# phecda-xu/FullyCNNSpeechEnhancement

Measured on AMD Instinct MI355X. Metric: spectrogram frames/sec (CR-CED-16 fwd, 129-bin), higher is better.
Workload: dtype f32; 1 GPU; CR-CED V3 (16-layer, skip connections) forward, batch 256 per GPU, 129x512, fp32 (BASELINE configs[2]); variant=FullyCNNV3, batch_per_gpu=256, frames=512, bins=129, global_batch=256, fused_available=True, parallelism=batch-shard x1, rccl_world_size=1, weights=random-init (glorot, seed 42), library=rced-hip 0.1 gfx950

## Files before the change

fullycnnspeechenhancement_amd/csrc/kernels_fused_v3.h:

```cpp
#pragma once
#include <hip/hip_runtime.h>

#include <type_traits>

#include "lds_dma.h"

#ifndef RCED_V3_LEGACY_FORMS
#define RCED_V3_LEGACY_FORMS 0
#endif
#ifndef RCED_D1
#define RCED_D1 1
#endif
#ifndef RCED_D2
#define RCED_D2 2
#endif
#ifndef RCED_D2X
#define RCED_D2X 1
#endif
#ifndef RCED_D3
#define RCED_D3 2
#endif
#ifndef RCED_LANE_OPAQUE
#define RCED_LANE_OPAQUE 1
#endif
// ... 1168 lines not shown
  constexpr int kPadPairs = 64 * kHS / 2;
#pragma unroll
  for (int i = 0; i < (5 * kPadPairs + kThreads - 1) / kThreads; ++i) {
    const int q = tid + i * kThreads, p = q / kPadPairs, e = q - p * kPadPairs;
    if (q < 5 * kPadPairs) lds_st<f32x2>(lds0 + 4 * (M::kHOff + p * kHFrame * kHS + 2 * e), 0, f32x2{0.f, 0.f});
  }
}
typedef f32x4 __attribute__((aligned(4))) f32x4_u;
template <int CTRL>
__device__ __forceinline__ float row_dpp(float v) {
  return __builtin_bit_cast(float, __builtin_amdgcn_update_dpp(0, __builtin_bit_cast(int, v), CTRL, 0xf, 0xf, true));
}

template <class M>
__device__ __forceinline__ void final_phase(const Params& P, unsigned lds0, unsigned w128, int wave, int lane, int utt,
                                            int t0, const FinA& A, const XStage& xnext, float* x0) {
  lane = opaque(lane);
  const int n = lane & 15, kq = lane >> 4;
  const f32x4 zero4 = {0.f, 0.f, 0.f, 0.f};
  float* yt = P.y + ((size_t)utt * P.T + t0) * kF;
  const int nfr = P.T - t0 < kTF ? P.T - t0 : kTF;
  if (wave == 2) {
    const int fi = kq, sub = n;
    const unsigned hb = lds0 + 4 * (M::kHOff + (kHFrame * fi + 64 + 64 + sub) * kHS);
    const unsigned wb = w128 + sub * 32;
    f32x4 hv[5][2], wv[5][2];
#pragma unroll
    for (int m = 0; m < 5; ++m)
#pragma unroll
      for (int c = 0; c < 2; ++c) {
        const f32x2 h0 = lds_ld<f32x2>(hb, (16 * m * kHS + 4 * c) * 4), h1 = lds_ld<f32x2>(hb, (16 * m * kHS + 4 * c + 2) * 4);
        hv[m][c] = f32x4{h0.x, h0.y, h1.x, h1.y};
        wv[m][c] = lds_ld<f32x4>(wb, (16 * m * 8 + 4 * c) * 4);
      }
    f32x4 s4 = {0.f, 0.f, 0.f, 0.f};
#pragma unroll
    for (int m = 0; m < 5; ++m)
#pragma unroll
      for (int c = 0; c < 2; ++c) {
        s4.x = __builtin_fmaf(hv[m][c].x, wv[m][c].x, s4.x);
        s4.y = __builtin_fmaf(hv[m][c].y, wv[m][c].y, s4.y);
        s4.z = __builtin_fmaf(hv[m][c].z, wv[m][c].z, s4.z);
        s4.w = __builtin_fmaf(hv[m][c].w, wv[m][c].w, s4.w);
      }
    float sum = (s4.x + s4.y) + (s4.z + s4.w);
    sum += row_dpp<0xB1>(sum);
    sum += row_dpp<0x4E>(sum);
    sum += row_dpp<0x141>(sum);
    sum += row_dpp<0x140>(sum);
    if (sub == 0 && fi < nfr) yt[fi * kF + 128] = sum + P.fin_bias;
  }
  {
    const unsigned rd0 = lds0 + 4 * (M::kHOff + ((kHFrame * (n >> 2) + 16 * (n & 3)) * kHS + 2 * kq)) + wave * (kFinRun * kHS * 4);
    unsigned rd1 = rd0 + 64 * kHS * 4;
    asm volatile("" : "+v"(rd1));
    f32x4 acc[2][2] = {{zero4, zero4}, {zero4, zero4}};
    constexpr int D = 2, RING = D + 1;
    f32x2 b[RING][2];
    run_job<kFinRun, D>(
        [&](auto ic) {
          constexpr int i = decltype(ic)::value, r = i % RING;
          b[r][0] = lds_ld<f32x2>(rd0, i * kHS * 4);
          b[r][1] = lds_ld<f32x2>(rd1, i * kHS * 4);
        },
        [&](auto ic) {
          constexpr int i = decltype(ic)::value, r = i % RING;
          acc[0][0] = mfma(A.a[i].x, b[r][0].x, acc[0][0]);
          acc[1][0] = mfma(A.a[i].x, b[r][1].x, acc[1][0]);
          acc[0][1] = mfma(A.a[i].y, b[r][0].y, acc[0][1]);
          acc[1][1] = mfma(A.a[i].y, b[r][1].y, acc[1][1]);
        },
        [] {});
    const unsigned scr = lds0 + M::finscr0(wave) + lane * 16;
    lds_st<f32x4>(scr, 0, acc[0][0] + acc[0][1]);
    lds_st<f32x4>(scr, M::kFinScrCt, acc[1][0] + acc[1][1]);
  }
  xstage_store(xnext, x0, wave * 64 + lane);
  __syncthreads();
  if (wave < 2) {
    const unsigned scr = lds0 + wave * M::kFinScrCt + lane * 16;
    f32x4 v = lds_ld<f32x4>(scr, M::finscr0(0));
#pragma unroll
    for (int w = 1; w < kWaves; ++w) v += lds_ld<f32x4>(scr, M::finscr0(w));
    v += f32x4{P.fin_bias, P.fin_bias, P.fin_bias, P.fin_bias};
    const int fi = n >> 2, f0 = 16 * (4 * wave + (n & 3)) + 4 * kq;
    if (fi < nfr) {
      *reinterpret_cast<f32x4_u*>(yt + fi * kF + f0) = v;
      store_wait_state();
    }
  } else if (wave == 3 && !M::kFused) {
    if constexpr (M::kX6) {
      constexpr int kRows = kB18Pad + 4 * kTF;
#pragma unroll
      for (int i = 0; i < (3 * kRows * 2 + 63) / 64; ++i) {
        const int q = lane + 64 * i, pl = q / (kRows * 2), e = q - pl * (kRows * 2), rr = e >> 1, half = e & 1;
        const int row = rr < kB18Pad ? rr : kB18Pad + kF + kS * ((rr - kB18Pad) >> 2) + ((rr - kB18Pad) & 3);
        if (q < 3 * kRows * 2) lds_st<f32x4>(lds0 + 4 * M::kB18Off + pl * M::kPlaneBytes + row * 32 + half * 16, 0, zero4);
      }
    } else {
      constexpr int kGapPairs = 4 * 18 / 2;
#pragma unroll
      for (int i = 0; i < (4 * kGapPairs + 63) / 64; ++i) {
        const int q = lane + 64 * i, g = q / kGapPairs, e = q - g * kGapPairs;
        if (q < 4 * kGapPairs)
          lds_st<f32x2>(lds0 + 4 * (M::kB18Off + (kB18Pad + kF + kS * g) * 18 + 2 * e), 0, f32x2{0.f, 0.f});
      }
    }
  }
}

#include "kernels_fused_v3_allx6.h"

template <class M>
__global__ __launch_bounds__(RCED_V3_LB) __attribute__((target("no-packed-fp32-ops"))) void fused_v3_kernel(Params P) {
  extern __shared__ __attribute__((aligned(16))) float lds[];
  const int tid = threadIdx.x;
  const int lane = tid & 63;
  const int wave = __builtin_amdgcn_readfirstlane(tid >> 6);
  float* const wbase = lds + M::kWOff;
#define WREG(i) (wbase + (i) * kWRegion)

  for (int e = tid; e < M::kLdsFloats; e += kThreads) lds[e] = 0.f;
  __syncthreads();
  A1Regs A1;
  A2Regs A2;
  const wrsrc_t wrs = __builtin_amdgcn_make_buffer_rsrc(const_cast<float*>(P.wpack), 0, (M::kAllX6 ? kATotal : M::kFused ? kTTotal : M::kX6 ? kGTotal : kWTotal) * 4, 0x00020000);
  constexpr bool kL1X = M::kFused && RCED_T_L1X6;
  auto wload = [&](auto kc, int g, unsigned voff, int g1size = kG1) {
    constexpr int k = decltype(kc)::value;
    if constexpr (k < 7) a1_load_one<k>(A1, wrs, g, voff);
    else if constexpr (k < 17) a2_load_one<k - 7>(A2, wrs, g + g1size, RCED_L2_BOTH ? 0 : wave >> 2, voff);
  };
  if constexpr (M::kAllX6) {
    packet_dma<kFinTFloats>(P.fin, lds + M::kFinTOff, wave, lane);
    a1x_dma<M>(P.wpack, lds, wave, lane);
  } else if constexpr (M::kX6) {
    const unsigned voff = (unsigned)lane * 16u;
    static_for<0, 7>([&](auto kc) { wload(kc, 0, voff); });
    if constexpr (M::kFused) packet_dma<kFin128>(P.fin + kFinA, lds + M::kFin128Off, wave, lane);
  } else {
    packet_dma<kW1>(P.wpack, WREG(0), wave, lane);
  }
  int wcur = 0;
  unsigned epoch = 0;
  const int tiles_base = P.total_tiles / (int)gridDim.x, tiles_rem = P.total_tiles % (int)gridDim.x;
  const int tile_begin = (int)blockIdx.x * tiles_base + ((int)blockIdx.x < tiles_rem ? (int)blockIdx.x : tiles_rem);
  const int tile_end = tile_begin + tiles_base + ((int)blockIdx.x < tiles_rem ? 1 : 0);
  XStage xst = xstage_load(P, tile_begin < tile_end ? tile_begin : P.total_tiles, tid);
#if RCED_STAMPS
  unsigned long long tsum[8] = {0, 0, 0, 0, 0, 0, 0, 0}, tfin = 0, tdet[16] = {0, 0, 0, 0, 0, 0, 0, 0, 0, 0, 0, 0, 0, 0, 0, 0};
#endif
  layer_end_sync();

  const int w1 = M::kFused && RCED_T_L1SWAP ? wave ^ 4 : wave;
  const int xr0 = w1 == 7 ? 3 : w1 - 4;
#ifdef RCED_PRIO
  if ((wave >= 4) == (RCED_PRIO > 0)) __builtin_amdgcn_s_setprio(1);
#endif
  const Lane L = make_lane<M>(lds, wave, lane, xr0 < 0 ? 0 : xr0, w1);
  const unsigned lds0 = lds_addr(lds);
  xstage_store(xst, lds + M::kX0Off, tid);
  __syncthreads();
  if constexpr (M::kAllX6) {
    convert_x0<M>(lds0, wave, lane);
    __syncthreads();
  }
  constexpr int kBlockFloats = M::kFused ? kTBlock : M::kX6 ? kGBlock : kWBlock;

  for (int tile = tile_begin; tile < tile_end; ++tile) {
    const int utt = tile / P.tiles_per_utt;
    const int t0 = (tile - utt * P.tiles_per_utt) * kTF;
    f32x4 skip_ce1[3], skip_ce2[3];
#pragma unroll
    for (int t = 0; t < 3; ++t) skip_ce1[t] = skip_ce2[t] = f32x4{0.f, 0.f, 0.f, 0.f};
    f32x2 sk1[5], sk2[5];
#pragma unroll
    for (int t = 0; t < 5; ++t) sk1[t] = sk2[t] = f32x2{0.f, 0.f};
    const float* wsrc = P.wpack;
    int gofs = 0;

    auto l1_section = [&](auto whichc, int blk) __attribute__((always_inline)) {
      constexpr int which = decltype(whichc)::value;
      {
        STAMP_BEGIN();
        const unsigned wb = lds_addr(WREG(wcur));
        auto dma = [&] {
          if constexpr (M::kFused) packet_dma<kG2 + kW3T>(wsrc + (M::kAllX6 ? kG1A : kL1X && blk > 0 ? kG1X : kG1), WREG(0), wave, lane);
          else if constexpr (M::kX6) packet_dma<kW3>(wsrc + kG1 + kG2, WREG(0), wave, lane);
          else packet_dma<kW2>(wsrc + kW1, WREG(wcur ^ 1), wave, lane);
        };
        A1Rem A1r;
        const unsigned voff1 = (unsigned)opaque(lane) * 16u;
        auto sp1 = [&](auto kc) {
          constexpr int k = decltype(kc)::value;
          if constexpr (M::kX6 && !(RCED_X6_EXP & 2)) {
            if constexpr (k >= 10) a1_load_rem_one<k - 10>(A1r, wrs, gofs, voff1);
            else if constexpr (!M::kFused || ((RCED_T_A2REG == 1 || RCED_T_A2REG == 2) && k < 9)) wload(IC<k + 7>{}, gofs, voff1);
          }
        };
        auto late = [&] {
          if constexpr (M::kX6 && (!M::kFused || RCED_T_A2REG == 2) && RCED_L2_BOTH && !(RCED_X6_EXP & 2))
            static_for<0, 10>([&](auto kc) { a2_load_one<decltype(kc)::value, kL2MT - 1>(A2, wrs, gofs + kG1, 1, voff1); });
        };
        auto sp1x = [&](auto kc) {
          constexpr int k = decltype(kc)::value;
          if constexpr (kL1X && k >= 12 && k < 21 && (RCED_T_A2REG == 1 || RCED_T_A2REG == 2)) wload(IC<k - 12 + 7>{}, gofs, voff1, M::kAllX6 ? kG1A : kG1X);
        };
        if constexpr (kL1X) {
          if constexpr (which == 1) layer1<M, true>(L, wb, A1, A1r, w1, dma, sp1, late DET_PASS);
          else layer1_x6l<M>(L, lds0, w1, dma, sp1x DET_PASS);
        } else {
          if (blk == 0) layer1<M, true>(L, wb, A1, A1r, w1, dma, sp1, late DET_PASS);
          else layer1<M, false>(L, wb, A1, A1r, w1, dma, sp1, late DET_PASS);
        }

        if constexpr (!M::kX6) wcur ^= 1;
#if RCED_STAMPS
        const unsigned long long st_b_ = stamp();
        tsum[blk == 0 ? 6 : 0] += st_b_ - st_a_;
        layer_end_sync();
        tsum[blk == 0 ? 7 : 3] += stamp() - st_b_;
#else
        layer_end_sync();
#endif
        if constexpr (!M::kFused) {
          STAMP_BEGIN();
          const unsigned tag2 = 0xC0000000u | (epoch + 1u);
          if constexpr (M::kX6) {
#if RCED_V3_LEGACY_FORMS
            if constexpr (RCED_L2_BOTH) layer2_x6_both<M>(L, lds0, A2, wave, tag2, P.err, [] {} DET_PASS);
            else layer2_x6<M>(L, lds0, A2, wave, tag2, P.err, [] {} DET_PASS);
#else
            static_assert(!M::kX6 || M::kFused, "form 1 is a legacy form (RCED_V3_LEGACY_FORMS)");
#endif
          } else {
            auto dma3 = [&] { packet_dma<kW3>(wsrc + kW1 + kW2, WREG(wcur ^ 1), wave, lane); };
            layer2_f32<M>(L, lds0, lds_addr(WREG(wcur)), wave, tag2, P.err, dma3 DET_PASS);
            wcur ^= 1;
          }
          STAMP_MATH(1);
          layer_end_sync();
          STAMP_WAIT(1);
        }
            }
    };
    if constexpr (M::kAllX6) l1_section(IC<0>{}, 0);
    else if constexpr (kL1X) l1_section(IC<1>{}, 0);
#pragma unroll 1
    for (int blk = 0;; ++blk) {
      if constexpr (kL1X) {
        if (blk > 0) l1_section(IC<0>{}, blk);
      } else {
        l1_section(IC<2>{}, blk);
      }
      if (blk == 4) break;
      if constexpr (M::kFused) {
        STAMP_BEGIN();
        ++epoch;
        const unsigned voff = (unsigned)opaque(lane) * 16u;
        auto sp = [&](auto jc) {
          constexpr int j = decltype(jc)::value;
          if constexpr (!kL1X) {
            if constexpr (2 * j < 7) wload(IC<2 * j>{}, gofs + kBlockFloats, voff);
            if constexpr (2 * j + 1 < 7) wload(IC<2 * j + 1>{}, gofs + kBlockFloats, voff);
          }
        };
        auto dma1 = [&] {
          if constexpr (kL1X) a1x_dma<M>(wsrc + (M::kAllX6 ? kTBlockA : blk == 0 ? kTBlock : kTBlockX), lds, wave, lane);
        };
        layer23<M, false>(P, L, lds0, lds_addr(WREG(0)), A2, blk, wave, 0x80000000u | epoch, sk1, sk2, sp, dma1 DET_PASS);
        STAMP_MATH(2);
        layer_end_sync();
        STAMP_WAIT(2);
      } else {
        STAMP_BEGIN();
        const unsigned wb = lds_addr(WREG(M::kX6 ? 0 : wcur));
        ++epoch;
        const unsigned tag = 0x80000000u | epoch;
        const float* wnext = wsrc + kBlockFloats;
        auto dma = [&] {
          if constexpr (!M::kX6) packet_dma<kW1>(wnext, WREG(wcur ^ 1), wave, lane);
        };
        const unsigned voff = (unsigned)opaque(lane) * 16u;
        auto sp = [&](auto kc) {
          if constexpr (M::kX6 && !(RCED_X6_EXP & 4) && decltype(kc)::value < 7) wload(kc, gofs + kBlockFloats, voff);
        };
        layer3<M, false>(P, L, lds0, wb, blk, wave, tag, skip_ce1, skip_ce2, dma, sp DET_PASS);
        if constexpr (!M::kX6) wcur ^= 1;
        STAMP_MATH(2);
        layer_end_sync();
        STAMP_WAIT(2);
      }
      wsrc += M::kAllX6 ? kTBlockA : kL1X && blk > 0 ? kTBlockX : kBlockFloats;
      gofs += M::kAllX6 ? kTBlockA : kL1X && blk > 0 ? kTBlockX : kBlockFloats;
    }
    FinA finA;
    if constexpr (M::kAllX6) {
      STAMP_BEGIN();
      ++epoch;
      xst = xstage_load(P, tile + 1 < tile_end ? tile + 1 : P.total_tiles, tid);
      if (wave == 0 && lane < 3) lds_st<u32x4>(lds0 + 4 * M::kB8Off + kHZeroRow * 16 + (unsigned)lane * kHPlaneBytes, 0, u32x4{0u, 0u, 0u, 0u});
      auto dma1 = [&] { a1x_dma<M>(P.wpack, lds, wave, lane); };
      layer23<M, true>(P, L, lds0, lds_addr(WREG(0)), A2, 4, wave, 0x80000000u | epoch, sk1, sk2, [](auto) {}, dma1 DET_PASS);
      STAMP_MATH(2);
      layer_end_sync();
      STAMP_WAIT(2);
    } else if constexpr (M::kFused) {
      STAMP_BEGIN();
      ++epoch;
      xst = xstage_load(P, tile + 1 < tile_end ? tile + 1 : P.total_tiles, tid);
      const int lane_o = opaque(lane);
      auto sp = [&](auto jc) {
        constexpr int j = decltype(jc)::value, s0 = (kFinRun * j) / 5, s1 = (kFinRun * (j + 1)) / 5;
        const f32x2* src = reinterpret_cast<const f32x2*>(P.fin) + (size_t)(kFinRun * wave) * 64 + lane_o;
#pragma unroll
        for (int q = s0; q < s1; ++q) finA.a[q] = src[q * 64];
      };
      layer23<M, true>(P, L, lds0, lds_addr(WREG(0)), A2, 4, wave, 0x80000000u | epoch, sk1, sk2, sp, [] {} DET_PASS);
      STAMP_MATH(2);
      layer_end_sync();
      STAMP_WAIT(2);
      const unsigned voff = (unsigned)opaque(lane) * 16u;
      static_for<0, 7>([&](auto kc) { wload(kc, 0, voff); });
    } else {
      STAMP_BEGIN();
      const unsigned wb = lds_addr(WREG(M::kX6 ? 0 : wcur));
      ++epoch;
      const unsigned tag = 0x80000000u | epoch;
      xst = xstage_load(P, tile + 1 < tile_end ? tile + 1 : P.total_tiles, tid);
      if constexpr (M::kX6) packet_dma<kFin128>(P.fin + kFinA, lds + M::kFin128Off, wave, lane);
      else packet_dma<kFin128>(P.fin + kFinA, WREG(wcur ^ 1) + kW1, wave, lane);
      fin_prefetch(P, wave, lane, finA);
      fin_zero_pads<M>(lds0, tid);
      auto dma = [&] {
        if constexpr (!M::kX6) packet_dma<kW1>(P.wpack, WREG(wcur ^ 1), wave, lane);
      };
      const unsigned voff = (unsigned)opaque(lane) * 16u;
      auto sp = [&](auto kc) {
        if constexpr (M::kX6 && !(RCED_X6_EXP & 4) && decltype(kc)::value < 7) wload(kc, 0, voff);
      };
      layer3<M, true>(P, L, lds0, wb, 4, wave, tag, skip_ce1, skip_ce2, dma, sp DET_PASS);
      if constexpr (!M::kX6) wcur ^= 1;
      STAMP_MATH(2);
      layer_end_sync();
      STAMP_WAIT(2);
    }
#if RCED_STAMPS
    const unsigned long long st_f_ = stamp();
#endif
    if constexpr (M::kAllX6) {
      final_phase_x6<M>(P, lds0, wave, lane, utt, t0, xst, lds + M::kX0Off DET_PASS);
    } else {
      const unsigned w128 = M::kX6 ? lds0 + 4 * M::kFin128Off : lds_addr(WREG(wcur) + kW1);
      final_phase<M>(P, lds0, w128, wave, lane, utt, t0, finA, xst, lds + M::kX0Off);
    }
#if RCED_STAMPS
    tfin += stamp() - st_f_;
#endif
  }
#undef WREG
#if RCED_STAMPS
  if (P.stamps && blockIdx.x == 0 && lane == 0)
    for (int i = 0; i < 8; ++i) P.stamps[wave * 8 + i] = tsum[i];
  if (P.stamps && blockIdx.x == 0 && lane == 0) P.stamps[64 + wave * 3] = tfin;
  if (P.stamps && blockIdx.x == 0 && lane == 0)
    for (int i = 0; i < 16; ++i) P.stamps[88 + wave * 16 + i] = tdet[i];
#endif
}


}
}
```

fullycnnspeechenhancement_amd/csrc/kernels_fused_v3_allx6.h:

```cpp
#pragma once

template <class M>
__device__ __forceinline__ void convert_px(unsigned lds0, int i, int f) {
  const unsigned src = lds0 + 4 * (M::kX0Off + 4 + i * kS + f);
  float v[8];
#pragma unroll
  for (int rr = 0; rr < 8; ++rr) v[rr] = lds_ld<float>(src, rr * kS * 4);
  u32x4 h, m, l;
#pragma unroll
  for (int q = 0; q < 4; ++q) {
    const P3 p = split2(v[2 * q], v[2 * q + 1]);
    h[q] = p.h;
    m[q] = p.m;
    l[q] = p.l;
  }
  const unsigned dst = lds0 + 4 * M::kB8Off + (kB8Pad + i * kS + f) * 16;
  lds_st<u32x4>(dst, 0, h);
  lds_st<u32x4>(dst, kB8PlaneBytes, m);
  lds_st<u32x4>(dst, 2 * kB8PlaneBytes, l);
}
template <class M>
__device__ __forceinline__ void convert_x0(unsigned lds0, int wave, int lane) {
  lane = opaque(lane);
  const int tid = wave * 64 + lane;
  convert_px<M>(lds0, tid >> 7, tid & 127);
  if (wave == 7 && lane < kTF) convert_px<M>(lds0, lane, kF - 1);
  const int z = tid - 5 * 64;
  if (z >= 0 && z < 72) {
    const int part = z / 24, rr = z - part * 24;
    const int row = rr < 4 ? rr : rr < 20 ? kB8Pad + kS * ((rr - 4) >> 2) + kF + ((rr - 4) & 3) : kB8Pad + kNPX + (rr - 20);
    lds_st<u32x4>(lds0 + 4 * M::kB8Off + part * kB8PlaneBytes + row * 16, 0, u32x4{0u, 0u, 0u, 0u});
  }
}
static_assert(kB8Rows == kB8Pad + kNPX + 4, "convert_x0 zeroes the planes' pad, gap and trailing rows by this map");

template <class M, int NCH, bool CT2ALL>
__device__ __forceinline__ void fin_run(unsigned ra, unsigned ta, int b0, int b2, int q0, bool ct2first, unsigned zaddr, f32x4 (&acc)[3]) {
  s16x8 a[2][3];
  Parts b[2][3];
  auto ld = [&](auto ic) {
    constexpr int i = decltype(ic)::value, r = i & 1;
    const int q = q0 + i;
    const unsigned ta_i = ta + (unsigned)(64 * q);
#pragma unroll
    for (int p = 0; p < 3; ++p) a[r][p] = lds_ld<s16x8>(ta_i, p * kFinTPart);
    const unsigned ra_i = ra + (unsigned)(16 * (4 * q + (q >> 2)));
    const int bq = b0 + 4 * q;
#pragma unroll
    for (int ct = 0; ct < 3; ++ct) {
      if (ct == 2 && !(CT2ALL || i == 0)) continue;
      const bool ok = ct < 2 ? (unsigned)(bq + 64 * ct) <= 128u : (unsigned)(b2 + 4 * q) <= 128u;
      const unsigned ad = ok ? ra_i + 1088u * ct : zaddr;
      b[r][ct].h = lds_ld<s16x8>(ad, 0);
      b[r][ct].m = lds_ld<s16x8>(ad, kHPlaneBytes);
      b[r][ct].l = lds_ld<s16x8>(ad, 2 * kHPlaneBytes);
    }
  };
  ld(IC<0>{});
  pin();
  static_for<0, NCH>([&](auto ic) {
    constexpr int i = decltype(ic)::value, r = i & 1;
    if constexpr (i + 1 < NCH) ld(IC<i + 1>{});
    pin();
    mma2(a[r], b[r][0], acc[0], a[r], b[r][1], acc[1]);
    if constexpr (CT2ALL) {
      acc[2] = l2x_mma(a[r], b[r][2], acc[2]);
    } else if constexpr (i == 0) {
      if (ct2first) acc[2] = l2x_mma(a[r], b[r][2], acc[2]);
    }
    pin();
  });
}

template <class M>
__device__ __forceinline__ void final_phase_x6(const Params& P, unsigned lds0, int wave, int lane, int utt, int t0, const XStage& xnext, float* x0 DET_ARG) {
  DET_BEGIN();
  lane = opaque(lane);
  const int n = lane & 15, kq = lane >> 4;
  const f32x4 zero4 = {0.f, 0.f, 0.f, 0.f};
  float* yt = P.y + ((size_t)utt * P.T + t0) * kF;
  const int nfr = P.T - t0 < kTF ? P.T - t0 : kTF;
  xstage_store(xnext, x0, wave * 64 + lane);
  {
    const int fi = n >> 2, j0 = n & 3;
    const int b0 = 16 * j0 - 64 + kq;
    const int b2 = j0 == 0 ? b0 + 128 : 0x40000000;
    const unsigned ra = lds0 + 4 * M::kB8Off + (unsigned)((kHFr * fi + 17 * j0 - 68 + kq) * 16);
    const unsigned ta = lds0 + 4 * M::kFinTOff + (unsigned)((kq - n + 15) * 16);
    const unsigned zaddr = lds0 + 4 * M::kB8Off + kHZeroRow * 16;
    f32x4 acc[3] = {zero4, zero4, zero4};
    if (wave < 4) {
      fin_run<M, 4, true>(ra, ta, b0, b2, 4 * wave, false, zaddr, acc);
    } else {
      const int run = 11 - wave;
      fin_run<M, 5, false>(ra, ta, b0, b2, 16 + 5 * (run - 4), run == 4, zaddr, acc);
    }
    const unsigned scr = lds0 + (unsigned)M::finscr(wave, 0) + (unsigned)lane * 16u;
#pragma unroll
    for (int ct = 0; ct < 3; ++ct) lds_st<f32x4>(scr, ct * M::kPlaneBytes, acc[ct]);
  }
  DET(8);
  __syncthreads();
  DET(9);
  if (wave < 3) {
    const unsigned scr = lds0 + (unsigned)(M::finscr(0, 0) + wave * M::kPlaneBytes) + (unsigned)lane * 16u;
    f32x4 v = lds_ld<f32x4>(scr, 0);
#pragma unroll
    for (int w = 1; w < kWaves; ++w) v += lds_ld<f32x4>(scr, M::finscr(w, 0) - M::finscr(0, 0));
    v += f32x4{P.fin_bias, P.fin_bias, P.fin_bias, P.fin_bias};
    const int fi = n >> 2;
    if (wave < 2) {
      const int f0 = 16 * (4 * wave + (n & 3)) + 4 * kq;
      if (fi < nfr) {
        *reinterpret_cast<f32x4_u*>(yt + fi * kF + f0) = v;
        store_wait_state();
      }
    } else if (kq == 0 && (n & 3) == 0 && fi < nfr) {
      yt[fi * kF + kF - 1] = v.x;
    }
  }
  DET(10);
  convert_x0<M>(lds0, wave, lane);
  DET(11);
  __syncthreads();
  DET(12);
}
```

Before: 23.82 million frames/s.

## Overlap next-tile input conversion with final-layer MMAs and rebalance final-phase work

The next tile's input staging store moves ahead of the last layer-end barrier. The fp32-to-split-bf16 conversion of the next input is then interleaved into the final 1x-conv MMA loops: its reads are issued before the loop and its splits in the loop bodies, and only the plane stores remain after the reduction. Final-phase work is redistributed into fin_run3 and fin_run2 schedules, with the ct=2 column spread across waves, and the cross-wave reduction loads are batched before summing. The aim is to hide conversion and load latency behind matrix ops, at the cost of more register pressure and a more complex per-wave mapping.

Result: no change. 23.81 million frames/s (-0.0%).

```diff
diff --git a/fullycnnspeechenhancement_amd/csrc/kernels_fused_v3.h b/fullycnnspeechenhancement_amd/csrc/kernels_fused_v3.h
--- a/fullycnnspeechenhancement_amd/csrc/kernels_fused_v3.h
+++ b/fullycnnspeechenhancement_amd/csrc/kernels_fused_v3.h
@@ -1494,6 +1494,7 @@
       if (wave == 0 && lane < 3) lds_st<u32x4>(lds0 + 4 * M::kB8Off + kHZeroRow * 16 + (unsigned)lane * kHPlaneBytes, 0, u32x4{0u, 0u, 0u, 0u});
       auto dma1 = [&] { a1x_dma<M>(P.wpack, lds, wave, lane); };
       layer23<M, true>(P, L, lds0, lds_addr(WREG(0)), A2, 4, wave, 0x80000000u | epoch, sk1, sk2, [](auto) {}, dma1 DET_PASS);
+      xstage_store(xst, lds + M::kX0Off, tid);
       STAMP_MATH(2);
       layer_end_sync();
       STAMP_WAIT(2);
@@ -1541,7 +1542,7 @@
     const unsigned long long st_f_ = stamp();
 #endif
     if constexpr (M::kAllX6) {
-      final_phase_x6<M>(P, lds0, wave, lane, utt, t0, xst, lds + M::kX0Off DET_PASS);
+      final_phase_x6<M>(P, lds0, wave, lane, utt, t0 DET_PASS);
     } else {
       const unsigned w128 = M::kX6 ? lds0 + 4 * M::kFin128Off : lds_addr(WREG(wcur) + kW1);
       final_phase<M>(P, lds0, w128, wave, lane, utt, t0, finA, xst, lds + M::kX0Off);
diff --git a/fullycnnspeechenhancement_amd/csrc/kernels_fused_v3_allx6.h b/fullycnnspeechenhancement_amd/csrc/kernels_fused_v3_allx6.h
--- a/fullycnnspeechenhancement_amd/csrc/kernels_fused_v3_allx6.h
+++ b/fullycnnspeechenhancement_amd/csrc/kernels_fused_v3_allx6.h
@@ -1,30 +1,42 @@
 #pragma once
 
-template <class M>
-__device__ __forceinline__ void convert_px(unsigned lds0, int i, int f) {
+struct PxIn {
+  float v[8];
+};
+struct PxOut {
+  u32x4 h, m, l;
+};
+template <class M>
+__device__ __forceinline__ void px_read(unsigned lds0, int i, int f, PxIn& in) {
   const unsigned src = lds0 + 4 * (M::kX0Off + 4 + i * kS + f);
-  float v[8];
-#pragma unroll
-  for (int rr = 0; rr < 8; ++rr) v[rr] = lds_ld<float>(src, rr * kS * 4);
-  u32x4 h, m, l;
-#pragma unroll
-  for (int q = 0; q < 4; ++q) {
-    const P3 p = split2(v[2 * q], v[2 * q + 1]);
-    h[q] = p.h;
-    m[q] = p.m;
-    l[q] = p.l;
-  }
+  if (RCED_T_EXP & 131072) return;
+#pragma unroll
+  for (int rr = 0; rr < 8; ++rr) in.v[rr] = lds_ld<float>(src, rr * kS * 4);
+}
+template <int Q>
+__device__ __forceinline__ void px_split(const PxIn& in, PxOut& o) {
+  if (RCED_T_EXP & 131072) {
+    o.h[Q] = 0x3f803f80u;
+    o.m[Q] = o.l[Q] = 0u;
+    return;
+  }
+  const P3 p = split2(in.v[2 * Q], in.v[2 * Q + 1]);
+  o.h[Q] = p.h;
+  o.m[Q] = p.m;
+  o.l[Q] = p.l;
+}
+template <class M>
+__device__ __forceinline__ void px_store(unsigned lds0, int i, int f, const PxOut& o) {
   const unsigned dst = lds0 + 4 * M::kB8Off + (kB8Pad + i * kS + f) * 16;
-  lds_st<u32x4>(dst, 0, h);
-  lds_st<u32x4>(dst, kB8PlaneBytes, m);
-  lds_st<u32x4>(dst, 2 * kB8PlaneBytes, l);
-}
-template <class M>
-__device__ __forceinline__ void convert_x0(unsigned lds0, int wave, int lane) {
-  lane = opaque(lane);
+  lds_st<u32x4>(dst, 0, o.h);
+  lds_st<u32x4>(dst, kB8PlaneBytes, o.m);
+  lds_st<u32x4>(dst, 2 * kB8PlaneBytes, o.l);
+}
+template <class M>
+__device__ __forceinline__ void planes_store(unsigned lds0, int wave, int lane, const PxOut& pa, const PxOut& pb) {
   const int tid = wave * 64 + lane;
-  convert_px<M>(lds0, tid >> 7, tid & 127);
-  if (wave == 7 && lane < kTF) convert_px<M>(lds0, lane, kF - 1);
+  px_store<M>(lds0, tid >> 7, tid & 127, pa);
+  if (wave >= 4 && lane == 0) px_store<M>(lds0, wave - 4, kF - 1, pb);
   const int z = tid - 5 * 64;
   if (z >= 0 && z < 72) {
     const int part = z / 24, rr = z - part * 24;
@@ -32,68 +44,150 @@
     lds_st<u32x4>(lds0 + 4 * M::kB8Off + part * kB8PlaneBytes + row * 16, 0, u32x4{0u, 0u, 0u, 0u});
   }
 }
-static_assert(kB8Rows == kB8Pad + kNPX + 4, "convert_x0 zeroes the planes' pad, gap and trailing rows by this map");
+static_assert(kB8Rows == kB8Pad + kNPX + 4, "planes_store zeroes the planes' pad, gap and trailing rows by this map");
+static_assert(kTF == 4 && kWaves == 8, "bin 128 of frame f is wave 4 + f's");
+template <class M>
+__device__ __forceinline__ void convert_x0(unsigned lds0, int wave, int lane) {
+  lane = opaque(lane);
+  const int tid = wave * 64 + lane;
+  PxIn ia, ib;
+  PxOut pa, pb;
+  px_read<M>(lds0, tid >> 7, tid & 127, ia);
+  static_for<0, 4>([&](auto qc) { px_split<decltype(qc)::value>(ia, pa); });
+  if (wave >= 4) {
+    px_read<M>(lds0, wave - 4, kF - 1, ib);
+    static_for<0, 4>([&](auto qc) { px_split<decltype(qc)::value>(ib, pb); });
+  } else {
+    pb = pa;
+  }
+  planes_store<M>(lds0, wave, lane, pa, pb);
+}
 
-template <class M, int NCH, bool CT2ALL>
-__device__ __forceinline__ void fin_run(unsigned ra, unsigned ta, int b0, int b2, int q0, bool ct2first, unsigned zaddr, f32x4 (&acc)[3]) {
-  s16x8 a[2][3];
+struct FinLane {
+  unsigned ra, ta, zaddr;
+  int b0, b2;
+};
+template <int CT>
+__device__ __forceinline__ void fin_ldb(const FinLane& F, int q, Parts& p) {
+  const int bq = (CT < 2 ? F.b0 + 64 * CT : F.b2) + 4 * q;
+  const unsigned ad = (unsigned)bq <= 128u ? F.ra + (unsigned)(16 * (4 * q + (q >> 2)) + 1088 * CT) : F.zaddr;
+  p.h = lds_ld<s16x8>(ad, 0);
+  p.m = lds_ld<s16x8>(ad, kHPlaneBytes);
+  p.l = lds_ld<s16x8>(ad, 2 * kHPlaneBytes);
+}
+__device__ __forceinline__ void fin_lda(const FinLane& F, int q, s16x8 (&a)[3]) {
+  const unsigned t = F.ta + (unsigned)(64 * q);
+#pragma unroll
+  for (int p = 0; p < 3; ++p) a[p] = lds_ld<s16x8>(t, p * kFinTPart);
+}
+template <int NM, int NV, class PRE, class SP>
+__device__ __forceinline__ void fin_run3(const FinLane& F, int qv0, int qu0, int qu3, f32x4 (&acc)[3], PRE&& pre, SP&& sp) {
+  s16x8 au[2][3], av[2][3];
   Parts b[2][3];
   auto ld = [&](auto ic) {
     constexpr int i = decltype(ic)::value, r = i & 1;
-    const int q = q0 + i;
-    const unsigned ta_i = ta + (unsigned)(64 * q);
-#pragma unroll
-    for (int p = 0; p < 3; ++p) a[r][p] = lds_ld<s16x8>(ta_i, p * kFinTPart);
-    const unsigned ra_i = ra + (unsigned)(16 * (4 * q + (q >> 2)));
-    const int bq = b0 + 4 * q;
-#pragma unroll
-    for (int ct = 0; ct < 3; ++ct) {
-      if (ct == 2 && !(CT2ALL || i == 0)) continue;
-      const bool ok = ct < 2 ? (unsigned)(bq + 64 * ct) <= 128u : (unsigned)(b2 + 4 * q) <= 128u;
-      const unsigned ad = ok ? ra_i + 1088u * ct : zaddr;
-      b[r][ct].h = lds_ld<s16x8>(ad, 0);
-      b[r][ct].m = lds_ld<s16x8>(ad, kHPlaneBytes);
-      b[r][ct].l = lds_ld<s16x8>(ad, 2 * kHPlaneBytes);
+    const int qv = qv0 + i, qu = i == 3 ? qu3 : qu0 + i;
+    fin_lda(F, qu, au[r]);
+    fin_lda(F, qv, av[r]);
+    fin_ldb<0>(F, qu, b[r][0]);
+    fin_ldb<1>(F, qv, b[r][1]);
+    if (!(RCED_T_EXP & 65536)) fin_ldb<2>(F, qv, b[r][2]);
+  };
+  ld(IC<0>{});
+  pre();
+  pin();
+  static_for<0, 4>([&](auto ic) {
+    constexpr int i = decltype(ic)::value, r = i & 1;
+    if constexpr (i + 1 < 4) ld(IC<i + 1>{});
+    pin();
+    mma2(au[r], b[r][0], acc[0], av[r], b[r][1], acc[1]);
+    if (!(RCED_T_EXP & 65536)) acc[2] = l2x_mma(av[r], b[r][2], acc[2]);
+    sp(ic);
+    interleave<NM, NV>();
+    pin();
+  });
+}
+template <int NM, int NV, class PRE, class SP>
+__device__ __forceinline__ void fin_run2(const FinLane& F, int q0, bool extra, f32x4 (&acc)[3], PRE&& pre, SP&& sp) {
+  s16x8 a[2][3];
+  Parts b[2][2];
+  auto ld = [&](auto ic) {
+    constexpr int i = decltype(ic)::value, r = i & 1;
+    if constexpr (i < 4) {
+      fin_lda(F, q0 + i, a[r]);
+      fin_ldb<0>(F, q0 + i, b[r][0]);
+      fin_ldb<1>(F, q0 + i, b[r][1]);
+    } else if (!(RCED_T_EXP & 65536)) {
+      fin_lda(F, 16, a[r]);
+      fin_ldb<1>(F, 16, b[r][0]);
+      fin_ldb<2>(F, 16, b[r][1]);
     }
   };
   ld(IC<0>{});
+  pre();
   pin();
-  static_for<0, NCH>([&](auto ic) {
-    constexpr int i = decltype(ic)::value, r = i & 1;
-    if constexpr (i + 1 < NCH) ld(IC<i + 1>{});
+  static_for<0, 4>([&](auto ic) {
+    constexpr int i = decltype(ic)::value, r = i & 1;
+    ld(IC<i + 1>{});
     pin();
     mma2(a[r], b[r][0], acc[0], a[r], b[r][1], acc[1]);
-    if constexpr (CT2ALL) {
-      acc[2] = l2x_mma(a[r], b[r][2], acc[2]);
-    } else if constexpr (i == 0) {
-      if (ct2first) acc[2] = l2x_mma(a[r], b[r][2], acc[2]);
-    }
+    sp(ic);
+    interleave<NM, NV>();
     pin();
   });
+  if (!(RCED_T_EXP & 65536)) {
+    if (extra) mma2(a[0], b[0][0], acc[1], a[0], b[0][1], acc[2]);
+    pin();
+  }
 }
 
 template <class M>
-__device__ __forceinline__ void final_phase_x6(const Params& P, unsigned lds0, int wave, int lane, int utt, int t0, const XStage& xnext, float* x0 DET_ARG) {
+__device__ __forceinline__ void final_phase_x6(const Params& P, unsigned lds0, int wave, int lane, int utt, int t0 DET_ARG) {
   DET_BEGIN();
   lane = opaque(lane);
-  const int n = lane & 15, kq = lane >> 4;
+  const int n = lane & 15, kq = lane >> 4, tid = wave * 64 + lane;
   const f32x4 zero4 = {0.f, 0.f, 0.f, 0.f};
   float* yt = P.y + ((size_t)utt * P.T + t0) * kF;
   const int nfr = P.T - t0 < kTF ? P.T - t0 : kTF;
-  xstage_store(xnext, x0, wave * 64 + lane);
+  PxIn ia, ib;
+  PxOut pa, pb;
   {
     const int fi = n >> 2, j0 = n & 3;
-    const int b0 = 16 * j0 - 64 + kq;
-    const int b2 = j0 == 0 ? b0 + 128 : 0x40000000;
-    const unsigned ra = lds0 + 4 * M::kB8Off + (unsigned)((kHFr * fi + 17 * j0 - 68 + kq) * 16);
-    const unsigned ta = lds0 + 4 * M::kFinTOff + (unsigned)((kq - n + 15) * 16);
-    const unsigned zaddr = lds0 + 4 * M::kB8Off + kHZeroRow * 16;
+    FinLane F;
+    F.b0 = 16 * j0 - 64 + kq;
+    F.b2 = j0 == 0 ? F.b0 + 128 : 0x40000000;
+    F.ra = lds0 + 4 * M::kB8Off + (unsigned)((kHFr * fi + 17 * j0 - 68 + kq) * 16);
+    F.ta = lds0 + 4 * M::kFinTOff + (unsigned)((kq - n + 15) * 16);
+    F.zaddr = lds0 + 4 * M::kB8Off + kHZeroRow * 16;
     f32x4 acc[3] = {zero4, zero4, zero4};
     if (wave < 4) {
-      fin_run<M, 4, true>(ra, ta, b0, b2, 4 * wave, false, zaddr, acc);
+      auto pre = [&] { px_read<M>(lds0, tid >> 7, tid & 127, ia); };
+      auto sp = [&](auto ic) {
+        constexpr int i = decltype(ic)::value;
+        if constexpr (i == 1 || i == 2) {
+          px_split<2 * i - 2>(ia, pa);
+          px_split<2 * i - 1>(ia, pa);
+        }
+      };
+      const bool w3 = wave == 3;
+      fin_run3<12, 2>(F, w3 ? 0 : 4 + 4 * wave, w3 ? 33 : 4 + 4 * wave, w3 ? 16 : 7 + 4 * wave, acc, pre, sp);
+      pb = pa;
     } else {
-      const int run = 11 - wave;
-      fin_run<M, 5, false>(ra, ta, b0, b2, 16 + 5 * (run - 4), run == 4, zaddr, acc);
+      auto pre = [&] {
+        px_read<M>(lds0, tid >> 7, tid & 127, ia);
+        px_read<M>(lds0, (tid >> 6) - 4, kF - 1, ib);
+      };
+      auto sp = [&](auto ic) {
+        constexpr int i = decltype(ic)::value;
+        if constexpr (i < 2) {
+          px_split<2 * i>(ia, pa);
+          px_split<2 * i + 1>(ia, pa);
+        } else {
+          px_split<2 * i - 4>(ib, pb);
+          px_split<2 * i - 3>(ib, pb);
+        }
+      };
+      fin_run2<8, 3>(F, 17 + 4 * (wave - 4), wave == 4, acc, pre, sp);
     }
     const unsigned scr = lds0 + (unsigned)M::finscr(wave, 0) + (unsigned)lane * 16u;
 #pragma unroll
@@ -104,9 +198,13 @@
   DET(9);
   if (wave < 3) {
     const unsigned scr = lds0 + (unsigned)(M::finscr(0, 0) + wave * M::kPlaneBytes) + (unsigned)lane * 16u;
-    f32x4 v = lds_ld<f32x4>(scr, 0);
-#pragma unroll
-    for (int w = 1; w < kWaves; ++w) v += lds_ld<f32x4>(scr, M::finscr(w, 0) - M::finscr(0, 0));
+    f32x4 part[kWaves];
+#pragma unroll
+    for (int w = 0; w < kWaves; ++w) part[w] = lds_ld<f32x4>(scr, M::finscr(w, 0) - M::finscr(0, 0));
+    pin();
+    f32x4 v = part[0];
+#pragma unroll
+    for (int w = 1; w < kWaves; ++w) v += part[w];
     v += f32x4{P.fin_bias, P.fin_bias, P.fin_bias, P.fin_bias};
     const int fi = n >> 2;
     if (wave < 2) {
@@ -120,7 +218,7 @@
     }
   }
   DET(10);
-  convert_x0<M>(lds0, wave, lane);
+  planes_store<M>(lds0, wave, lane, pa, pb);
   DET(11);
   __syncthreads();
   DET(12);
```
